# kartikmadhira1/YA_VO

Hardware: AMD Instinct MI355X
Metric: frames/sec (detect+describe+match+PnP) on 1241×376 KITTI stereo; RMSE vs CPU ref (higher is better)
Workload: dtype u8

## Files before the change

ya_vo_amd/csrc/yavo_kernels.hip:

```cpp
#include <hip/hip_runtime.h>
#include <stdint.h>
#include <stdlib.h>
#include <string.h>

#include <algorithm>

#include "yavo_xlane.h"
#include "yavo_internal.h"


namespace yavo {

__device__ __forceinline__ int lane_id() { return (int)(threadIdx.x & 63); }

__device__ __forceinline__ int wave_incl_scan(int v) {
    v += __builtin_amdgcn_update_dpp(0, v, 0x111, 0xf, 0xf, false);
    v += __builtin_amdgcn_update_dpp(0, v, 0x112, 0xf, 0xf, false);
    v += __builtin_amdgcn_update_dpp(0, v, 0x114, 0xf, 0xf, false);
    v += __builtin_amdgcn_update_dpp(0, v, 0x118, 0xf, 0xf, false);
    v += __builtin_amdgcn_update_dpp(0, v, 0x142, 0xa, 0xf, false);
    v += __builtin_amdgcn_update_dpp(0, v, 0x143, 0xc, 0xf, false);
    return v;
}

// ... 162 lines not shown
    return kw;
}

__device__ __forceinline__ int reflect101(int p, int len) {
    if (p < 0) p = -p;
    if (p >= len) p = 2 * len - p - 2;
    return p;
}

#ifdef YAVO_LM_PROFILE
constexpr int kDetProfSlots = 131072;
__device__ unsigned long long g_det_prof[kDetProfSlots][6];
#define DP_DECL unsigned long long dp_acc[6] = {0, 0, 0, 0, 0, 0}; unsigned long long dp_t = __builtin_readcyclecounter();
#define DP_MARK(k) do { const unsigned long long t_ = __builtin_readcyclecounter(); dp_acc[k] += t_ - dp_t; dp_t = t_; } while (0)
#define DP_STORE() do { \
        const unsigned slot_ = blockIdx.x; \
        if (threadIdx.x == 0 && slot_ < kDetProfSlots) for (int q_ = 0; q_ < 6; ++q_) g_det_prof[slot_][q_] = dp_acc[q_]; \
    } while (0)
constexpr int kBriefProfSlots = 16384;
__device__ unsigned long long g_brief_prof[kBriefProfSlots][6];
#define BP_DECL unsigned long long bp_acc[3] = {0, 0, 0}; unsigned long long bp_t = __builtin_readcyclecounter(); \
    unsigned long long bp_bands = 0; const unsigned long long bp_rt0 = __builtin_amdgcn_s_memrealtime();
#define BP_MARK(k) do { const unsigned long long t_ = __builtin_readcyclecounter(); bp_acc[k] += t_ - bp_t; bp_t = t_; } while (0)
#define BP_BAND() do { ++bp_bands; } while (0)
#define BP_STORE() do { \
        if (threadIdx.x == 0 && blockIdx.x < kBriefProfSlots) { \
            g_brief_prof[blockIdx.x][0] = bp_acc[0]; g_brief_prof[blockIdx.x][1] = bp_acc[1]; \
            g_brief_prof[blockIdx.x][2] = bp_rt0; \
            g_brief_prof[blockIdx.x][3] = __builtin_amdgcn_s_memrealtime(); \
            g_brief_prof[blockIdx.x][4] = (unsigned long long)__builtin_amdgcn_s_getreg(0xF804) | (bp_bands << 32); \
            g_brief_prof[blockIdx.x][5] = (unsigned long long)__builtin_amdgcn_s_getreg(0xF814) | (bp_acc[2] << 32); \
        } \
    } while (0)
#else
#define DP_DECL
#define DP_MARK(k) do {} while (0)
#define DP_STORE() do {} while (0)
#define BP_DECL
#define BP_MARK(k) do {} while (0)
#define BP_BAND() do {} while (0)
#define BP_STORE() do {} while (0)
#endif
constexpr int FT_W = kFastTileW;
constexpr int FT_H = kFastTileH;
constexpr int FT_R = 4;
constexpr int FT_LW = FT_W + 2 * FT_R;
constexpr int FT_LH = FT_H + 2 * FT_R;
constexpr int kBandM = 19;
constexpr int kBlurStageDw = FT_LH * (FT_W / 4);

__device__ __forceinline__ void blur_tile_mfma(const uint8_t* tile, const uint32_t* s_band, uint32_t* stage, int hbias,
                                               int lane, int cb) {
    typedef int dt_v4i __attribute__((ext_vector_type(4)));
    const int nn = lane & 15, g = lane >> 4;
    const uint32_t* band = &s_band[(nn & 3) * kBandM + 3 - (nn >> 2)];
    const dt_v4i B = {(int)band[4 * g], (int)band[4 * g + 1], (int)band[4 * g + 2], (int)band[4 * g + 3]};
    const dt_v4i Z = {0, 0, 0, 0};
    const uint8_t* arow = &tile[nn * FT_LW + 16 * cb + 16 * g];
    dt_v4i Hlo, Hhi;
#pragma unroll
    for (int rb = 0; rb < 4; ++rb) {
        const uint2 lo = *reinterpret_cast<const uint2*>(arow + 16 * rb * FT_LW);
        const uint2 hi = *reinterpret_cast<const uint2*>(arow + 16 * rb * FT_LW + 8);
        const dt_v4i A = {(int)(lo.x ^ 0x80808080u), (int)(lo.y ^ 0x80808080u), (int)(hi.x ^ 0x80808080u),
                          (int)(hi.y ^ 0x80808080u)};
        const dt_v4i acc = __builtin_amdgcn_mfma_i32_16x16x64_i8(A, B, Z, 0, 0, 0);
        const uint32_t p01 = __builtin_amdgcn_perm((uint32_t)acc[1], (uint32_t)acc[0], 0x05010400u);
        const uint32_t p23 = __builtin_amdgcn_perm((uint32_t)acc[3], (uint32_t)acc[2], 0x05010400u);
        Hlo[rb] = (int)(__builtin_amdgcn_perm(p23, p01, 0x05040100u) ^ 0x80808080u);
        Hhi[rb] = (int)__builtin_amdgcn_perm(p23, p01, 0x07060302u);
// ... 280 lines not shown
    for (int rr = ty; rr < BL_H; rr += 4) {
        const int r = r0 + rr;
        uint32_t acc = 0;
#pragma unroll
        for (int i = 0; i < 9; ++i) acc += kw.k[i] * th[(rr + i) * BL_W + tx];
        uint32_t v = (acc + (1u << 15)) >> 16;
        if (r < H && c < W) blur[(int64_t)img * blur_image_bytes(H, W) + (int64_t)r * blur_pitch(W) + c] = (uint8_t)(v > 255u ? 255u : v);
    }
}

void launch_blur9(const uint8_t* imgs, int n_images, int H, int W, int stride, int64_t pitch,
                  const uint16_t* k9_host, uint8_t* blur, hipStream_t s) {
    const K9 kw = make_k9(k9_host);
    constexpr int kMaxGridZ = 65535;
    for (int i0 = 0; i0 < n_images; i0 += kMaxGridZ) {
        const int n = n_images - i0 < kMaxGridZ ? n_images - i0 : kMaxGridZ;
        dim3 grid((W + BL_W - 1) / BL_W, (H + BL_H - 1) / BL_H, n);
        hipLaunchKernelGGL(blur9_kernel, grid, dim3(256), 0, s, imgs + (int64_t)i0 * pitch, H, W, stride, pitch, kw,
                           blur + (int64_t)i0 * blur_image_bytes(H, W));
    }
}

constexpr int TK_NT = 1024;

__device__ __forceinline__ bool brief_boundary(int row, int col, int H, int W) {
    return !(col - 8 < 0 || col + 8 > W) && !(row - 8 < 0 || row + 8 > H);
}

__host__ __device__ constexpr int bank_classes(int nb) { return nb <= kBandCounters / 32 ? 32 : 1; }

template <int NT, class RcAt>
__device__ void boundary_compact(RcAt rc_at, int K, int H, int W, int32_t* kp_src, int32_t* kp_count,
                                 int32_t* kp_band, int32_t* band_off, int* s_tmp, int* s_band) {
    const int tid = threadIdx.x;
    const int nb = (H + kBandRows - 1) / kBandRows;
    const int C = bank_classes(nb), nbc = nb * C;
    const int LS = brief_lds_stride(W);
    auto bucket = [&](int row, int col) -> int {
        const int band = row / kBandRows;
        const int cls = C == 1 ? 0 : ((((row - band * kBandRows + 8) * LS + col) >> 2) & 31);
        return band * C + cls;
    };
    for (int b = tid; b < nbc; b += NT) s_band[b] = 0;
    __syncthreads();
    int base = 0;
    for (int pass = 0; pass < 2; ++pass) {
        base = 0;
        for (int c0 = 0; c0 < K; c0 += 4 * NT) {
            int flags[4];
            int2 rcs[4];
            int cnt = 0;
#pragma unroll
            for (int u = 0; u < 4; ++u) {
                const int i = c0 + tid * 4 + u;
                flags[u] = 0;
                rcs[u] = make_int2(0, 0);
                if (i < K) {
                    rcs[u] = rc_at(i);
                    flags[u] = brief_boundary(rcs[u].x, rcs[u].y, H, W) ? 1 : 0;
                }
                cnt += flags[u];
            }
            int total = 0;
            int off = base + block_excl_scan<NT>(cnt, s_tmp, &total);
#pragma unroll
            for (int u = 0; u < 4; ++u) {
                const int i = c0 + tid * 4 + u;
                if (flags[u]) {
                    const int bk = bucket(rcs[u].x, rcs[u].y);
                    if (pass == 0) {
                        reinterpret_cast<int4*>(kp_src)[off] = make_int4(rcs[u].x, rcs[u].y, i, 0);
                        atomicAdd(&s_band[bk], 1);
                    } else {
                        const int pos = atomicAdd(&s_band[bk], 1);
                        reinterpret_cast<int4*>(kp_band)[pos] = make_int4(rcs[u].x, rcs[u].y, i, off);
                    }
                    off++;
                }
            }
            base += total;
        }
        __syncthreads();
        if (pass == 0) {
            int acc = 0;
            for (int b0 = 0; b0 < nbc; b0 += NT) {
                const int j = b0 + tid;
                const int c = j < nbc ? s_band[j] : 0;
                int tot = 0;
                const int first = acc + block_excl_scan<NT>(c, s_tmp, &tot);
                if (j < nbc) {
                    s_band[j] = first;
                    if (j % C == 0) band_off[j / C] = first;
                }
                acc += tot;
            }
            if (tid == 0) band_off[nb] = acc;
        }
        __syncthreads();
    }
    if (tid == 0) *kp_count = base;
}

constexpr int TK_SEL_NT = 512;
static_assert(TK_SEL_NT >= 256 && TK_SEL_NT % 64 == 0, "the radix-select histogram scan uses the first 256 threads");
template <int NT>
__global__ __launch_bounds__(NT) void topk_kernel(const uint64_t* __restrict__ cand_keys, int64_t cap,
                                                     uint32_t* __restrict__ cand_count, uint32_t* __restrict__ cand_seen,
                                                     int H, int W, int max_kp, int keep, int32_t* __restrict__ det_rc,
                                                     float* __restrict__ det_resp, int32_t* __restrict__ det_count,
                                                     int32_t* __restrict__ kp_src, int32_t* __restrict__ kp_count,
                                                     int32_t* __restrict__ kp_band, int32_t* __restrict__ band_off,
                                                     int32_t* __restrict__ brief_heads) {
    __shared__ uint64_t s_keys[kMaxKp];
    __shared__ uint32_t s_hist[256];
    __shared__ int s_tmp[40];
    __shared__ int s_band[kBandCounters];
    __shared__ uint64_t s_prefix, s_mask;
    __shared__ int s_krem, s_done, s_n;

    const int img = blockIdx.x;
    const int tid = threadIdx.x;
    if (img == 0 && tid < kBriefHeads) brief_heads[tid] = 0;
    const uint64_t* keys = cand_keys + (int64_t)img * cap;
    int64_t C64 = (int64_t)cand_count[img];
    if (C64 > cap) C64 = cap;
    const int C = (int)C64;
    const int K = C < keep ? C : keep;
    __syncthreads();
    if (tid == 0) {
        cand_seen[img] = (uint32_t)C;
        cand_count[img] = 0;
    }
    int32_t* rc_out = det_rc + (int64_t)img * max_kp * 2;
    float* resp_out = det_resp + (int64_t)img * max_kp;

    if (K == 0) {
        const int nb = (H + kBandRows - 1) / kBandRows;
        for (int b = tid; b <= nb; b += NT) band_off[(int64_t)img * (kMaxBands + 1) + b] = 0;
        if (tid == 0) { det_count[img] = 0; kp_count[img] = 0; }
        return;
    }
    uint64_t sel_mask = 0, sel_prefix = ~0ull;
    if (C > K) {
        if (tid == 0) { s_prefix = 0; s_mask = 0; s_krem = K; s_done = 0; }
        __syncthreads();
        for (int shift = 56; shift >= 0; shift -= 8) {
            const uint64_t pm = s_mask, pp = s_prefix;
            const int krem = s_krem;
            if (tid < 256) s_hist[tid] = 0;
            __syncthreads();
            for (int i = tid; i < C; i += NT) {
                const uint64_t k = keys[i];
                if ((k & pm) == pp) atomicAdd(&s_hist[(k >> shift) & 255u], 1u);
            }
            __syncthreads();
            int h = 0, incl = 0;
            if (tid < 256) {
                h = (int)s_hist[tid];
                incl = wave_incl_scan(h);
                if ((tid & 63) == 63) s_tmp[tid >> 6] = incl;
            }
            __syncthreads();
            if (tid < 256) {
                int base = 0;
                for (int w = 0; w < (tid >> 6); ++w) base += s_tmp[w];
                incl += base;
                if (incl >= krem && incl - h < krem) {
                    const int nk = krem - (incl - h);
                    s_prefix = pp | ((uint64_t)tid << shift);
                    s_mask = pm | (0xFFull << shift);
                    s_krem = nk;
                    s_done = (h == nk);
                }
            }
            __syncthreads();
            if (s_done) break;
        }
        sel_mask = s_mask;
        sel_prefix = s_prefix;
    }
    if (tid == 0) s_n = 0;
    __syncthreads();
    for (int i = tid; i < C; i += NT) {
        const uint64_t k = keys[i];
        if ((k & sel_mask) <= sel_prefix) {
            const int p = atomicAdd(&s_n, 1);
            if (p < kMaxKp) s_keys[p] = k;
        }
    }
    __syncthreads();
    int P2 = 1;
    while (P2 < K) P2 <<= 1;
    for (int i = K + tid; i < P2; i += NT) s_keys[i] = ~0ull;
    __syncthreads();
    for (int size = 2; size <= P2; size <<= 1) {
        for (int stride = size >> 1; stride > 0; stride >>= 1) {
            for (int t = tid; t < (P2 >> 1); t += NT) {
                const int i = 2 * t - (t & (stride - 1));
                const int j = i + stride;
                const bool up = ((i & size) == 0);
                const uint64_t a = s_keys[i], b = s_keys[j];
                if ((a > b) == up) { s_keys[i] = b; s_keys[j] = a; }
            }
            __syncthreads();
        }
    }
    for (int i = tid; i < K; i += NT) {
        const uint64_t k = s_keys[i];
        const uint32_t idx = (uint32_t)k;
        const int row = (int)(idx / (uint32_t)W), col = (int)(idx - (uint32_t)row * (uint32_t)W);
        rc_out[2 * i] = row;
        rc_out[2 * i + 1] = col;
        resp_out[i] = key_resp(k);
    }
    if (tid == 0) det_count[img] = K;
    const uint32_t Wu = (uint32_t)W;
    auto rc_from_lds = [&](int i) -> int2 {
        const uint32_t idx = (uint32_t)s_keys[i];
        const uint32_t row = idx / Wu;
        return make_int2((int)row, (int)(idx - row * Wu));
    };
    boundary_compact<NT>(rc_from_lds, K, H, W, kp_src + (int64_t)img * max_kp * 4, kp_count + img,
                         kp_band + (int64_t)img * max_kp * 4, band_off + (int64_t)img * (kMaxBands + 1), s_tmp, s_band);
}

__global__ __launch_bounds__(TK_NT) void kp_boundary_kernel(const int32_t* __restrict__ det_rc,
                                                            const int32_t* __restrict__ det_count, int H, int W,
                                                            int max_kp, int32_t* __restrict__ kp_src,
                                                            int32_t* __restrict__ kp_count, int32_t* __restrict__ kp_band,
                                                            int32_t* __restrict__ band_off,
                                                            int32_t* __restrict__ brief_heads) {
    __shared__ int s_tmp[40];
    __shared__ int s_band[kBandCounters];
    const int img = blockIdx.x;
    if (img == 0 && threadIdx.x < kBriefHeads) brief_heads[threadIdx.x] = 0;
    int K = det_count[img];
    if (K > max_kp) K = max_kp;
    const int32_t* rc = det_rc + (int64_t)img * max_kp * 2;
    auto rc_from_global = [&](int i) -> int2 { return make_int2(rc[2 * i], rc[2 * i + 1]); };
    boundary_compact<TK_NT>(rc_from_global, K, H, W, kp_src + (int64_t)img * max_kp * 4, kp_count + img,
                            kp_band + (int64_t)img * max_kp * 4, band_off + (int64_t)img * (kMaxBands + 1), s_tmp,
                            s_band);
}

void launch_topk(const uint64_t* cand_keys, int64_t cap, uint32_t* cand_count, uint32_t* cand_seen, int n_images,
                 int H, int W, int max_kp, int keep, int32_t* det_rc, float* det_resp, int32_t* det_count, int32_t* kp_src,
                 int32_t* kp_count, int32_t* kp_band, int32_t* band_off, int32_t* brief_heads, hipStream_t s) {
    hipLaunchKernelGGL(topk_kernel<TK_SEL_NT>, dim3(n_images), dim3(TK_SEL_NT), 0, s, cand_keys, cap, cand_count,
                       cand_seen, H, W, max_kp, keep, det_rc, det_resp, det_count, kp_src, kp_count, kp_band, band_off,
                       brief_heads);
}

void launch_kp_boundary(const int32_t* det_rc, const int32_t* det_count, int n_images, int H, int W, int max_kp,
                        int32_t* kp_src, int32_t* kp_count, int32_t* kp_band, int32_t* band_off, int32_t* brief_heads,
                        hipStream_t s) {
    hipLaunchKernelGGL(kp_boundary_kernel, dim3(n_images), dim3(TK_NT), 0, s, det_rc, det_count, H, W, max_kp,
                       kp_src, kp_count, kp_band, band_off, brief_heads);
}


constexpr int BR_BAND = kBandRows;
constexpr int BR_ROWS = BR_BAND + 17;
constexpr int BR_NT = 1024;
constexpr int BR_NW = BR_NT / 64;
static_assert(4 * BR_NT >= kMaxKp, "brief_kernel loads at most 4 * BR_NT band records");

__device__ __forceinline__ int brief_take(int32_t* heads, int label, int total, int& at) {
    const int q = total >> 3, r = total & 7;
    while (at < kBriefHeads) {
        const int x = (label + at) & 7;
        const int len = q + (x < r ? 1 : 0);
        if (len > 0) {
            const int v = atomicAdd(&heads[x], 1);
            if (v < len) return (x < r ? x * (q + 1) : r * (q + 1) + (x - r) * q) + v;
        }
        ++at;
    }
    return -1;
}

// ... 861 lines not shown
        const int i = tid * 4 + u;
        flags[u] = (i < n && (int)src[(int64_t)i * REC_DW + 24] < lim) ? 1 : 0;
        cnt += flags[u];
    }
    int total = 0;
    int off = block_excl_scan<FZ_NT>(cnt, s_tmp, &total);
#pragma unroll
    for (int u = 0; u < 4; ++u) {
        const int i = tid * 4 + u;
        if (i < n) s_pos[i] = flags[u] ? off : -1;
        off += flags[u];
    }
    __syncthreads();
    uint32_t* dst = reinterpret_cast<uint32_t*>(out);
    for (int dw = tid; dw < n * REC_DW; dw += FZ_NT) {
        const int i = dw / REC_DW;
        const int f = dw - i * REC_DW;
        const int p = s_pos[i];
        if (p < 0) continue;
        uint32_t v = src[dw];
        if (f == 3 || f == 15) v = (v & ~0xFFu) | 1u;
        dst[(int64_t)p * REC_DW + f] = v;
    }
    if (tid == 0) *out_count = total;
}

void launch_filter_records(const yv_match* in, int n, int thr, yv_match* out, int32_t* out_count, hipStream_t s) {
    hipLaunchKernelGGL(filter_records_kernel, dim3(1), dim3(FZ_NT), 0, s, in, n, thr, out, out_count);
}

}

#ifdef YAVO_LM_PROFILE
extern "C" int yv_debug_brief_prof(unsigned long long* out ) {
    return hipMemcpyFromSymbol(out, HIP_SYMBOL(yavo::g_brief_prof), sizeof(unsigned long long) * 16384 * 6) ==
                   hipSuccess ? 0 : -2;
}
extern "C" int yv_debug_det_prof(unsigned long long* out ) {
    return hipMemcpyFromSymbol(out, HIP_SYMBOL(yavo::g_det_prof), sizeof(unsigned long long) * 131072 * 6) ==
                   hipSuccess ? 0 : -2;
}
#endif

namespace yavo {
__global__ void xlane_check_kernel(int32_t* out) {
    const int l = threadIdx.x;
    out[0 * 64 + l] = xl::xor_row_i32<1>(l);
    out[1 * 64 + l] = xl::xor_row_i32<2>(l);
    out[2 * 64 + l] = xl::xor_row_i32<4>(l);
    out[3 * 64 + l] = xl::xor_row_i32<8>(l);
    uint32_t a = (uint32_t)l, b = 100u + (uint32_t)l;
    xl::swap_halves<16>(a, b);
    out[4 * 64 + l] = (int32_t)a;
    out[5 * 64 + l] = (int32_t)b;
    a = (uint32_t)l;
    b = 100u + (uint32_t)l;
    xl::swap_halves<32>(a, b);
    out[6 * 64 + l] = (int32_t)a;
    out[7 * 64 + l] = (int32_t)b;
}
}

extern "C" int yv_debug_xlane(int32_t* d_out , void* stream) {
    if (!d_out) return -1;
    hipLaunchKernelGGL(yavo::xlane_check_kernel, dim3(1), dim3(64), 0, reinterpret_cast<hipStream_t>(stream), d_out);
    return hipGetLastError() == hipSuccess ? 0 : -2;
}
```

Baseline: 255,700.

## Add register-resident fast top-k kernel with wave-level radix select and bitonic sort

Adds a topk_fast_kernel that holds up to 16 candidate keys per thread in registers. It narrows the radix select with wave OR/AND reductions over the high key bits, builds per-wave ballot-peeled histograms, sorts four keys per thread with in-register cross-lane bitonic stages that go through LDS only for large strides, and fuses the boundary compaction and band scan. Its goal is to cut the many LDS passes and syncthreads of the generic shared-memory bitonic sort and select. Images with too many candidates fall back to the refactored general path. This adds a large amount of code and register pressure, with an occupancy attribute pinned to 8 waves per EU.

```diff
diff --git a/ya_vo_amd/csrc/yavo_kernels.hip b/ya_vo_amd/csrc/yavo_kernels.hip
--- a/ya_vo_amd/csrc/yavo_kernels.hip
+++ b/ya_vo_amd/csrc/yavo_kernels.hip
@@ -218,7 +218,22 @@
             g_brief_prof[blockIdx.x][5] = (unsigned long long)__builtin_amdgcn_s_getreg(0xF814) | (bp_acc[2] << 32); \
         } \
     } while (0)
+constexpr int kTopkProfSlots = 8192;
+__device__ unsigned long long g_topk_prof[kTopkProfSlots][8];
+#define TP_DECL unsigned long long tp_acc[6] = {0, 0, 0, 0, 0, 0}; unsigned long long tp_t = __builtin_readcyclecounter(); \
+    const unsigned long long tp_rt0 = __builtin_amdgcn_s_memrealtime();
+#define TP_MARK(k) do { const unsigned long long t_ = __builtin_readcyclecounter(); tp_acc[k] += t_ - tp_t; tp_t = t_; } while (0)
+#define TP_STORE() do { \
+        if (threadIdx.x == 0 && blockIdx.x < kTopkProfSlots) { \
+            for (int q_ = 0; q_ < 6; ++q_) g_topk_prof[blockIdx.x][q_] = tp_acc[q_]; \
+            g_topk_prof[blockIdx.x][6] = tp_rt0; \
+            g_topk_prof[blockIdx.x][7] = __builtin_amdgcn_s_memrealtime(); \
+        } \
+    } while (0)
 #else
+#define TP_DECL
+#define TP_MARK(k) do {} while (0)
+#define TP_STORE() do {} while (0)
 #define DP_DECL
 #define DP_MARK(k) do {} while (0)
 #define DP_STORE() do {} while (0)
@@ -640,19 +655,15 @@
 constexpr int TK_SEL_NT = 512;
 static_assert(TK_SEL_NT >= 256 && TK_SEL_NT % 64 == 0, "the radix-select histogram scan uses the first 256 threads");
 template <int NT>
-__global__ __launch_bounds__(NT) void topk_kernel(const uint64_t* __restrict__ cand_keys, int64_t cap,
-                                                     uint32_t* __restrict__ cand_count, uint32_t* __restrict__ cand_seen,
-                                                     int H, int W, int max_kp, int keep, int32_t* __restrict__ det_rc,
-                                                     float* __restrict__ det_resp, int32_t* __restrict__ det_count,
-                                                     int32_t* __restrict__ kp_src, int32_t* __restrict__ kp_count,
-                                                     int32_t* __restrict__ kp_band, int32_t* __restrict__ band_off,
-                                                     int32_t* __restrict__ brief_heads) {
-    __shared__ uint64_t s_keys[kMaxKp];
-    __shared__ uint32_t s_hist[256];
-    __shared__ int s_tmp[40];
-    __shared__ int s_band[kBandCounters];
-    __shared__ uint64_t s_prefix, s_mask;
-    __shared__ int s_krem, s_done, s_n;
+__device__ void topk_general(const uint64_t* __restrict__ cand_keys, int64_t cap, uint32_t* __restrict__ cand_count,
+                             uint32_t* __restrict__ cand_seen, int H, int W, int max_kp, int keep,
+                             int32_t* __restrict__ det_rc, float* __restrict__ det_resp,
+                             int32_t* __restrict__ det_count, int32_t* __restrict__ kp_src,
+                             int32_t* __restrict__ kp_count, int32_t* __restrict__ kp_band,
+                             int32_t* __restrict__ band_off, int32_t* __restrict__ brief_heads, uint64_t* s_keys,
+                             int key_cap, uint32_t* s_hist, int* s_tmp, int* s_band, uint64_t* s_state, int* s_ctl) {
+    uint64_t &s_prefix = s_state[0], &s_mask = s_state[1];
+    int &s_krem = s_ctl[0], &s_done = s_ctl[1], &s_n = s_ctl[2];
 
     const int img = blockIdx.x;
     const int tid = threadIdx.x;
@@ -721,7 +732,7 @@
         const uint64_t k = keys[i];
         if ((k & sel_mask) <= sel_prefix) {
             const int p = atomicAdd(&s_n, 1);
-            if (p < kMaxKp) s_keys[p] = k;
+            if (p < key_cap) s_keys[p] = k;
         }
     }
     __syncthreads();
@@ -758,6 +769,434 @@
     };
     boundary_compact<NT>(rc_from_lds, K, H, W, kp_src + (int64_t)img * max_kp * 4, kp_count + img,
                          kp_band + (int64_t)img * max_kp * 4, band_off + (int64_t)img * (kMaxBands + 1), s_tmp, s_band);
+}
+
+template <int NT>
+__global__ __launch_bounds__(NT) void topk_kernel(const uint64_t* __restrict__ cand_keys, int64_t cap,
+                                                     uint32_t* __restrict__ cand_count, uint32_t* __restrict__ cand_seen,
+                                                     int H, int W, int max_kp, int keep, int32_t* __restrict__ det_rc,
+                                                     float* __restrict__ det_resp, int32_t* __restrict__ det_count,
+                                                     int32_t* __restrict__ kp_src, int32_t* __restrict__ kp_count,
+                                                     int32_t* __restrict__ kp_band, int32_t* __restrict__ band_off,
+                                                     int32_t* __restrict__ brief_heads) {
+    __shared__ uint64_t s_keys[kMaxKp];
+    __shared__ uint32_t s_hist[256];
+    __shared__ int s_tmp[40];
+    __shared__ int s_band[kBandCounters];
+    __shared__ uint64_t s_state[2];
+    __shared__ int s_ctl[3];
+    topk_general<NT>(cand_keys, cap, cand_count, cand_seen, H, W, max_kp, keep, det_rc, det_resp, det_count, kp_src,
+                     kp_count, kp_band, band_off, brief_heads, s_keys, kMaxKp, s_hist, s_tmp, s_band, s_state, s_ctl);
+}
+
+constexpr int TKF_NT = 512;
+constexpr int TKF_R = 16;
+constexpr int TKF_CAP = TKF_NT * TKF_R;
+constexpr int TKF_MAXK = 4 * TKF_NT;
+constexpr int TKF_PEEL = 1;
+static_assert(TKF_NT * 16 == 8 * 256 * 4, "one 16-byte store per thread zeroes the eight histograms");
+static_assert(kBandCounters <= 2 * TKF_NT, "two (band, class) counters per thread");
+static_assert(kBriefHeads <= TKF_NT, "the band queue's heads are zeroed by one thread each");
+
+__device__ __forceinline__ uint64_t tk_u64(uint32_t lo, uint32_t hi) { return ((uint64_t)hi << 32) | lo; }
+
+__device__ __forceinline__ void tk_cx(uint64_t& a, uint64_t& b, bool up) {
+    const bool sw = (a > b) == up;
+    const uint64_t t = sw ? b : a;
+    b = sw ? a : b;
+    a = t;
+}
+
+template <int M>
+__device__ __forceinline__ void tk_lane_cx(uint64_t& k, bool keep_min) {
+    const uint32_t lo = (uint32_t)k, hi = (uint32_t)(k >> 32);
+    uint64_t a, b;
+    if constexpr (M < 16) {
+        a = k;
+        b = tk_u64(xl::xor_row<M>(lo), xl::xor_row<M>(hi));
+    } else {
+        uint32_t alo = lo, blo = lo, ahi = hi, bhi = hi;
+        xl::swap_halves<M>(alo, blo);
+        xl::swap_halves<M>(ahi, bhi);
+        a = tk_u64(alo, ahi);
+        b = tk_u64(blo, bhi);
+    }
+    k = ((a < b) == keep_min) ? a : b;
+}
+
+template <int STRIDE>
+__device__ __forceinline__ void tk_stage(uint64_t (&k)[4], bool up, int tid) {
+    if constexpr (STRIDE == 1) {
+        tk_cx(k[0], k[1], up);
+        tk_cx(k[2], k[3], up);
+    } else if constexpr (STRIDE == 2) {
+        tk_cx(k[0], k[2], up);
+        tk_cx(k[1], k[3], up);
+    } else {
+        constexpr int M = STRIDE / 4;
+        const bool keep_min = ((tid & M) == 0) == up;
+#pragma unroll
+        for (int j = 0; j < 4; ++j) tk_lane_cx<M>(k[j], keep_min);
+    }
+}
+template <int STRIDE>
+__device__ __forceinline__ void tk_merge(uint64_t (&k)[4], bool up, int tid) {
+    tk_stage<STRIDE>(k, up, tid);
+    if constexpr (STRIDE > 1) tk_merge<STRIDE / 2>(k, up, tid);
+}
+template <int SIZE>
+__device__ __forceinline__ void tk_sort_levels(uint64_t (&k)[4], int tid) {
+    if constexpr (SIZE == 2) {
+        tk_cx(k[0], k[1], true);
+        tk_cx(k[2], k[3], false);
+    } else {
+        tk_sort_levels<SIZE / 2>(k, tid);
+        tk_merge<SIZE / 2>(k, ((4 * tid) & SIZE) == 0, tid);
+    }
+}
+
+__device__ __forceinline__ uint32_t tk_wave_or(uint32_t v) {
+    v |= xl::xor_row<1>(v);
+    v |= xl::xor_row<2>(v);
+    v |= xl::xor_row<4>(v);
+    v |= xl::xor_row<8>(v);
+    uint32_t x = v, y = v;
+    xl::swap_halves<16>(x, y);
+    v = x | y;
+    x = y = v;
+    xl::swap_halves<32>(x, y);
+    return x | y;
+}
+
+__device__ __forceinline__ int tk_prefix_popc(uint64_t m) {
+    return (int)__builtin_amdgcn_mbcnt_hi((uint32_t)(m >> 32), __builtin_amdgcn_mbcnt_lo((uint32_t)m, 0u));
+}
+
+__device__ __forceinline__ void tk_hist_add(uint32_t* hist, uint32_t dg, bool act, int lane) {
+    bool pend = act;
+    if constexpr (TKF_PEEL > 0) {
+        uint64_t rem = __ballot(pend);
+#pragma unroll
+        for (int it = 0; it < TKF_PEEL; ++it) {
+            if (!rem) break;
+            const int src = __builtin_ctzll(rem);
+            const uint32_t d0 = (uint32_t)__builtin_amdgcn_readlane((int)dg, src);
+            const uint64_t same = __ballot(pend && dg == d0);
+            if (lane == src) atomicAdd(&hist[d0], (uint32_t)__builtin_popcountll(same));
+            pend = pend && dg != d0;
+            rem &= ~same;
+        }
+    }
+    if (pend) atomicAdd(&hist[dg], 1u);
+}
+template <bool LOW>
+__device__ __forceinline__ void tk_hist_pass(const uint64_t (&k)[TKF_R], uint32_t phi, uint32_t m, uint32_t p, int sh,
+                                             uint32_t* hist, int lane) {
+#pragma unroll
+    for (int r = 0; r < TKF_R; ++r) {
+        const uint32_t hi = (uint32_t)(k[r] >> 32), lo = (uint32_t)k[r];
+        const uint32_t w = LOW ? lo : hi;
+        const bool act = (w & m) == p && (!LOW || hi == phi);
+        tk_hist_add(hist, (w >> sh) & 255u, act, lane);
+    }
+}
+__device__ __forceinline__ void tk_find_bucket(const uint32_t* hist, int lane, int krem, int& bin, int& hh,
+                                               int& before) {
+    const uint4 h4 = reinterpret_cast<const uint4*>(hist)[lane];
+    const int h[4] = {(int)h4.x, (int)h4.y, (int)h4.z, (int)h4.w};
+    const int sum = h[0] + h[1] + h[2] + h[3];
+    const int incl = wave_incl_scan(sum);
+    int run = incl - sum, b = 0, c = 0, bf = 0;
+    const bool mine = run < krem && krem <= incl;
+#pragma unroll
+    for (int q = 0; q < 4; ++q) {
+        if (run < krem && krem <= run + h[q]) { b = 4 * lane + q; c = h[q]; bf = run; }
+        run += h[q];
+    }
+    const int src = __builtin_ctzll(__ballot(mine));
+    bin = __builtin_amdgcn_readlane(b, src);
+    hh = __builtin_amdgcn_readlane(c, src);
+    before = __builtin_amdgcn_readlane(bf, src);
+}
+
+#define TKF_OCCUPANCY __attribute__((amdgpu_waves_per_eu(8, 8)))
+template <int NT>
+__global__ __launch_bounds__(NT) TKF_OCCUPANCY void topk_fast_kernel(
+    const uint64_t* __restrict__ cand_keys, int64_t cap, uint32_t* __restrict__ cand_count,
+    uint32_t* __restrict__ cand_seen, int H, int W, int max_kp, int keep, int32_t* __restrict__ det_rc,
+    float* __restrict__ det_resp, int32_t* __restrict__ det_count, int32_t* __restrict__ kp_src,
+    int32_t* __restrict__ kp_count, int32_t* __restrict__ kp_band, int32_t* __restrict__ band_off,
+    int32_t* __restrict__ brief_heads, int force_general) {
+    static_assert(NT == TKF_NT, "the register layouts are written for 512 threads");
+    constexpr int NW = NT / 64;
+    __shared__ __attribute__((aligned(16))) uint64_t s_buf[2][TKF_MAXK];
+    __shared__ __attribute__((aligned(16))) int s_band[kBandCounters];
+    __shared__ __attribute__((aligned(16))) int s_tmp[40];
+    __shared__ uint64_t s_state[2];
+    __shared__ int s_ctl[3];
+    uint32_t* const s_hist = reinterpret_cast<uint32_t*>(s_buf[1]);
+
+    const int img = blockIdx.x;
+    const int tid = threadIdx.x, lane = tid & 63, wave = tid >> 6;
+    int64_t C64 = (int64_t)cand_count[img];
+    if (C64 > cap) C64 = cap;
+    const int C = (int)C64;
+    if (force_general || C > TKF_CAP) {
+        topk_general<NT>(cand_keys, cap, cand_count, cand_seen, H, W, max_kp, keep, det_rc, det_resp, det_count, kp_src,
+                         kp_count, kp_band, band_off, brief_heads, s_buf[0], TKF_MAXK, s_hist, s_tmp, s_band, s_state,
+                         s_ctl);
+        return;
+    }
+    const int K = C < keep ? C : keep;
+    if (img == 0 && tid < kBriefHeads) brief_heads[tid] = 0;
+    const int nb = (H + kBandRows - 1) / kBandRows;
+    int32_t* const boff = band_off + (int64_t)img * (kMaxBands + 1);
+    if (K == 0) {
+        __syncthreads();
+        for (int b = tid; b <= nb; b += NT) boff[b] = 0;
+        if (tid == 0) { cand_seen[img] = (uint32_t)C; cand_count[img] = 0; det_count[img] = 0; kp_count[img] = 0; }
+        return;
+    }
+
+    TP_DECL
+    const uint64_t* keys = cand_keys + (int64_t)img * cap;
+    uint64_t k[TKF_R];
+#pragma unroll
+    for (int r = 0; r < TKF_R; ++r) {
+        const int i = r * NT + tid;
+        k[r] = i < C ? keys[i] : ~0ull;
+    }
+    const int NC = bank_classes(nb), nbc = nb * NC;
+    reinterpret_cast<uint4*>(s_hist)[tid] = make_uint4(0u, 0u, 0u, 0u);
+    reinterpret_cast<uint4*>(s_buf[0])[2 * tid] = make_uint4(~0u, ~0u, ~0u, ~0u);
+    reinterpret_cast<uint4*>(s_buf[0])[2 * tid + 1] = make_uint4(~0u, ~0u, ~0u, ~0u);
+    for (int b = tid; b < nbc; b += NT) s_band[b] = 0;
+    if (tid == 0) s_ctl[2] = 0;
+    int P2 = 256;
+    while (P2 < K) P2 <<= 1;
+    const bool cut = C > P2;
+    if (cut) {
+        uint32_t o0 = 0u, a0 = ~0u, o1 = 0u, a1 = ~0u;
+        int n0 = 0;
+#pragma unroll
+        for (int r = 0; r < TKF_R; ++r) {
+            const uint32_t hi = (uint32_t)(k[r] >> 32);
+            const bool v = r * NT + tid < C, neg = (hi >> 31) != 0u;
+            n0 += __builtin_popcountll(__ballot(v && !neg));
+            o0 |= v && !neg ? hi : 0u;
+            a0 &= v && !neg ? hi : ~0u;
+            o1 |= v && neg ? hi : 0u;
+            a1 &= v && neg ? hi : ~0u;
+        }
+        o0 = tk_wave_or(o0);
+        a0 = ~tk_wave_or(~a0);
+        o1 = tk_wave_or(o1);
+        a1 = ~tk_wave_or(~a1);
+        if (lane == 0) {
+            int* t = s_tmp + 5 * wave;
+            t[0] = n0; t[1] = (int)o0; t[2] = (int)a0; t[3] = (int)o1; t[4] = (int)a1;
+        }
+    }
+    __syncthreads();
+    if (tid == 0) {
+        cand_seen[img] = (uint32_t)C;
+        cand_count[img] = 0;
+    }
+
+    TP_MARK(0);
+    uint64_t sel_mask = 0, sel_prefix = ~0ull;
+    if (cut) {
+        int n0 = 0;
+        uint32_t o0 = 0u, a0 = ~0u, o1 = 0u, a1 = ~0u;
+#pragma unroll
+        for (int w = 0; w < NW; ++w) {
+            const int* t = s_tmp + 5 * w;
+            n0 += t[0]; o0 |= (uint32_t)t[1]; a0 &= (uint32_t)t[2]; o1 |= (uint32_t)t[3]; a1 &= (uint32_t)t[4];
+        }
+        const bool c1 = K > n0;
+        int krem = __builtin_amdgcn_readfirstlane(c1 ? K - n0 : K);
+        const uint32_t orc = __builtin_amdgcn_readfirstlane(c1 ? o1 : o0);
+        const uint32_t andc = __builtin_amdgcn_readfirstlane(c1 ? a1 : a0);
+        const uint32_t diff = orc & ~andc;
+        const int hbh = diff ? 31 - __builtin_clz(diff) : -1;
+        uint32_t mhi = diff ? ~0u << (hbh + 1) : ~0u;
+        uint32_t phi = andc & mhi;
+        uint32_t mlo = 0u, plo = 0u;
+        int pass = 0, bin, hh, before, M;
+        bool done = false;
+        if (diff) {
+            for (int sh = hbh > 7 ? hbh - 7 : 0;; sh = sh > 8 ? sh - 8 : 0) {
+                uint32_t* hist = s_hist + 256 * pass++;
+                tk_hist_pass<false>(k, 0u, mhi, phi, sh, hist, lane);
+                __syncthreads();
+                tk_find_bucket(hist, lane, krem, bin, hh, before);
+                krem -= before;
+                phi |= (uint32_t)bin << sh;
+                mhi |= 0xFFu << sh;
+                M = K - krem + hh;
+                done = M <= P2;
+                if (done || sh == 0) break;
+            }
+        }
+        if (!done) {
+            for (int sh = 24;; sh = sh > 8 ? sh - 8 : 0) {
+                uint32_t* hist = s_hist + 256 * pass++;
+                tk_hist_pass<true>(k, phi, mlo, plo, sh, hist, lane);
+                __syncthreads();
+                tk_find_bucket(hist, lane, krem, bin, hh, before);
+                krem -= before;
+                plo |= (uint32_t)bin << sh;
+                mlo |= 0xFFu << sh;
+                M = K - krem + hh;
+                if (M <= P2 || sh == 0) break;
+            }
+        }
+        sel_mask = tk_u64(mlo, mhi);
+        sel_prefix = tk_u64(plo, phi);
+    }
+
+    TP_MARK(1);
+    {
+        uint32_t selbits = 0;
+        int wtot = 0;
+#pragma unroll
+        for (int r = 0; r < TKF_R; ++r) {
+            const bool s = (r * NT + tid < C) && (k[r] & sel_mask) <= sel_prefix;
+            selbits |= (s ? 1u : 0u) << r;
+            wtot += __builtin_popcountll(__ballot(s));
+        }
+        int base = 0;
+        if (lane == 0) base = atomicAdd(&s_ctl[2], wtot);
+        base = __builtin_amdgcn_readfirstlane(base);
+#pragma unroll
+        for (int r = 0; r < TKF_R; ++r) {
+            const bool s = (selbits >> r) & 1u;
+            const uint64_t bal = __ballot(s);
+            const int pos = base + tk_prefix_popc(bal);
+            if (s && pos < TKF_MAXK) s_buf[0][pos] = k[r];
+            base += __builtin_popcountll(bal);
+        }
+    }
+    __syncthreads();
+
+    TP_MARK(2);
+    uint64_t q[4] = {~0ull, ~0ull, ~0ull, ~0ull};
+    const bool live = 4 * tid < P2;
+    if (live) {
+        const uint4 a = reinterpret_cast<const uint4*>(s_buf[0])[2 * tid];
+        const uint4 b = reinterpret_cast<const uint4*>(s_buf[0])[2 * tid + 1];
+        q[0] = tk_u64(a.x, a.y); q[1] = tk_u64(a.z, a.w); q[2] = tk_u64(b.x, b.y); q[3] = tk_u64(b.z, b.w);
+        tk_sort_levels<256>(q, tid);
+    }
+    TP_MARK(3);
+    int cur = 1;
+    for (int size = 512; size <= P2; size <<= 1) {
+        const bool up = ((4 * tid) & size) == 0;
+        for (int stride = size >> 1; stride >= 256; stride >>= 1) {
+            if (live) {
+                uint4* dst = reinterpret_cast<uint4*>(s_buf[cur]) + 2 * tid;
+                dst[0] = make_uint4((uint32_t)q[0], (uint32_t)(q[0] >> 32), (uint32_t)q[1], (uint32_t)(q[1] >> 32));
+                dst[1] = make_uint4((uint32_t)q[2], (uint32_t)(q[2] >> 32), (uint32_t)q[3], (uint32_t)(q[3] >> 32));
+            }
+            __syncthreads();
+            if (live) {
+                const uint4* src = reinterpret_cast<const uint4*>(s_buf[cur]) + (((4 * tid) ^ stride) >> 1);
+                const uint4 a = src[0], b = src[1];
+                const uint64_t p[4] = {tk_u64(a.x, a.y), tk_u64(a.z, a.w), tk_u64(b.x, b.y), tk_u64(b.z, b.w)};
+                const bool keep_min = (((4 * tid) & stride) == 0) == up;
+#pragma unroll
+                for (int j = 0; j < 4; ++j) {
+                    q[j] = ((q[j] < p[j]) == keep_min) ? q[j] : p[j];
+                }
+            }
+            cur ^= 1;
+        }
+        if (live) tk_merge<128>(q, up, tid);
+    }
+
+    TP_MARK(4);
+    int32_t* rc_out = det_rc + (int64_t)img * max_kp * 2;
+    float* resp_out = det_resp + (int64_t)img * max_kp;
+    const uint32_t Wu = (uint32_t)W;
+    const int LS = brief_lds_stride(W);
+    int2 rcs[4];
+    int flags[4];
+    int cnt = 0;
+#pragma unroll
+    for (int j = 0; j < 4; ++j) {
+        const int i = 4 * tid + j;
+        flags[j] = 0;
+        rcs[j] = make_int2(0, 0);
+        if (i < K) {
+            const uint32_t idx = (uint32_t)q[j];
+            const uint32_t row = idx / Wu;
+            rcs[j] = make_int2((int)row, (int)(idx - row * Wu));
+            reinterpret_cast<int2*>(rc_out)[i] = rcs[j];
+            resp_out[i] = key_resp(q[j]);
+            flags[j] = brief_boundary(rcs[j].x, rcs[j].y, H, W) ? 1 : 0;
+        }
+        cnt += flags[j];
+    }
+    if (tid == 0) det_count[img] = K;
+    const int incl = wave_incl_scan(cnt);
+    if (lane == 63) s_tmp[8 + wave] = incl;
+    __syncthreads();
+    int off = incl - cnt, total = 0;
+#pragma unroll
+    for (int w = 0; w < NW; ++w) {
+        const int t = s_tmp[8 + w];
+        off += w < wave ? t : 0;
+        total += t;
+    }
+    int32_t* src_out = kp_src + (int64_t)img * max_kp * 4;
+    int32_t* band_out = kp_band + (int64_t)img * max_kp * 4;
+    int bks[4];
+#pragma unroll
+    for (int j = 0, o = off; j < 4; ++j) {
+        bks[j] = 0;
+        if (flags[j]) {
+            const int row = rcs[j].x, col = rcs[j].y;
+            const int band = row / kBandRows;
+            const int cls = NC == 1 ? 0 : ((((row - band * kBandRows + 8) * LS + col) >> 2) & 31);
+            bks[j] = band * NC + cls;
+            reinterpret_cast<int4*>(src_out)[o] = make_int4(row, col, 4 * tid + j, 0);
+            atomicAdd(&s_band[bks[j]], 1);
+            ++o;
+        }
+    }
+    __syncthreads();
+    {
+        const int j0 = 2 * tid;
+        const int c0 = j0 < nbc ? s_band[j0] : 0, c1 = j0 + 1 < nbc ? s_band[j0 + 1] : 0;
+        const int s = c0 + c1;
+        const int inc2 = wave_incl_scan(s);
+        if (lane == 63) s_tmp[16 + wave] = inc2;
+        __syncthreads();
+        int first = inc2 - s;
+#pragma unroll
+        for (int w = 0; w < NW; ++w) first += w < wave ? s_tmp[16 + w] : 0;
+        if (j0 < nbc) {
+            s_band[j0] = first;
+            if (j0 % NC == 0) boff[j0 / NC] = first;
+        }
+        if (j0 + 1 < nbc) {
+            s_band[j0 + 1] = first + c0;
+            if ((j0 + 1) % NC == 0) boff[(j0 + 1) / NC] = first + c0;
+        }
+        if (tid == 0) boff[nb] = total;
+    }
+    __syncthreads();
+#pragma unroll
+    for (int j = 0, o = off; j < 4; ++j) {
+        if (flags[j]) {
+            const int pos = atomicAdd(&s_band[bks[j]], 1);
+            reinterpret_cast<int4*>(band_out)[pos] = make_int4(rcs[j].x, rcs[j].y, 4 * tid + j, o);
+            ++o;
+        }
+    }
+    if (tid == 0) kp_count[img] = total;
+    TP_MARK(5);
+    TP_STORE();
 }
 
 __global__ __launch_bounds__(TK_NT) void kp_boundary_kernel(const int32_t* __restrict__ det_rc,
@@ -779,9 +1218,17 @@
                             s_band);
 }
 
+static int g_topk_path = 0;
+
 void launch_topk(const uint64_t* cand_keys, int64_t cap, uint32_t* cand_count, uint32_t* cand_seen, int n_images,
                  int H, int W, int max_kp, int keep, int32_t* det_rc, float* det_resp, int32_t* det_count, int32_t* kp_src,
                  int32_t* kp_count, int32_t* kp_band, int32_t* band_off, int32_t* brief_heads, hipStream_t s) {
+    if (max_kp <= TKF_MAXK && g_topk_path != 1) {
+        hipLaunchKernelGGL(topk_fast_kernel<TKF_NT>, dim3(n_images), dim3(TKF_NT), 0, s, cand_keys, cap, cand_count,
+                           cand_seen, H, W, max_kp, keep, det_rc, det_resp, det_count, kp_src, kp_count, kp_band,
+                           band_off, brief_heads, g_topk_path == 2 ? 1 : 0);
+        return;
+    }
     hipLaunchKernelGGL(topk_kernel<TK_SEL_NT>, dim3(n_images), dim3(TK_SEL_NT), 0, s, cand_keys, cap, cand_count,
                        cand_seen, H, W, max_kp, keep, det_rc, det_resp, det_count, kp_src, kp_count, kp_band, band_off,
                        brief_heads);
@@ -1709,6 +2156,10 @@
 }
 
 #ifdef YAVO_LM_PROFILE
+extern "C" int yv_debug_topk_prof(unsigned long long* out ) {
+    return hipMemcpyFromSymbol(out, HIP_SYMBOL(yavo::g_topk_prof), sizeof(unsigned long long) * 8192 * 8) ==
+                   hipSuccess ? 0 : -2;
+}
 extern "C" int yv_debug_brief_prof(unsigned long long* out ) {
     return hipMemcpyFromSymbol(out, HIP_SYMBOL(yavo::g_brief_prof), sizeof(unsigned long long) * 16384 * 6) ==
                    hipSuccess ? 0 : -2;
@@ -1718,6 +2169,13 @@
                    hipSuccess ? 0 : -2;
 }
 #endif
+
+extern "C" int yv_debug_set_topk_path(void* ctx, int mode) {
+    if (!ctx || mode < 0 || mode > 2) return -1;
+    yavo::g_topk_path = mode;
+    return 0;
+}
+extern "C" int yv_debug_topk_capacity(void) { return yavo::TKF_CAP; }
 
 namespace yavo {
 __global__ void xlane_check_kernel(int32_t* out) {
```

Result: no change. 257,400 (median of 3 runs) (+0.7%).

## Stage top-k radix select in LDS with adaptive bit passes and wave-aggregated compaction

Applied to the files above, without the earlier changes.

When the candidate count fits, the top-k select copies the 32-bit response keys into LDS once. It then runs the radix histogram passes from LDS, using AND/OR reductions to skip constant bits, rather than rereading global keys for every byte. Candidate gathering now uses one ballot-based atomic per wave instead of one atomic per thread. boundary_compact keeps its points in registers so it does not rerun the first pass, and sorted keys are repacked as row<<16|col to avoid integer division. The costs are more register and LDS pressure, extra profiling macros, and a fallback path for inputs too large to stage.

```diff
diff --git a/ya_vo_amd/csrc/yavo_kernels.hip b/ya_vo_amd/csrc/yavo_kernels.hip
--- a/ya_vo_amd/csrc/yavo_kernels.hip
+++ b/ya_vo_amd/csrc/yavo_kernels.hip
@@ -218,10 +218,20 @@
             g_brief_prof[blockIdx.x][5] = (unsigned long long)__builtin_amdgcn_s_getreg(0xF814) | (bp_acc[2] << 32); \
         } \
     } while (0)
+constexpr int kTopkProfSlots = 16384;
+__device__ unsigned long long g_topk_prof[kTopkProfSlots][5];
+#define TP_DECL unsigned long long tp_acc[5] = {0, 0, 0, 0, 0}; unsigned long long tp_t = __builtin_readcyclecounter();
+#define TP_MARK(k) do { const unsigned long long t_ = __builtin_readcyclecounter(); tp_acc[k] += t_ - tp_t; tp_t = t_; } while (0)
+#define TP_STORE() do { \
+        if (threadIdx.x == 0 && blockIdx.x < kTopkProfSlots) for (int q_ = 0; q_ < 5; ++q_) g_topk_prof[blockIdx.x][q_] = tp_acc[q_]; \
+    } while (0)
 #else
 #define DP_DECL
 #define DP_MARK(k) do {} while (0)
 #define DP_STORE() do {} while (0)
+#define TP_DECL
+#define TP_MARK(k) do {} while (0)
+#define TP_STORE() do {} while (0)
 #define BP_DECL
 #define BP_MARK(k) do {} while (0)
 #define BP_BAND() do {} while (0)
@@ -568,6 +578,8 @@
 template <int NT, class RcAt>
 __device__ void boundary_compact(RcAt rc_at, int K, int H, int W, int32_t* kp_src, int32_t* kp_count,
                                  int32_t* kp_band, int32_t* band_off, int* s_tmp, int* s_band) {
+    constexpr int NCH = (kMaxKp + 4 * NT - 1) / (4 * NT);
+    static_assert(NCH <= 2, "a thread keeps the points of all its chunks in registers");
     const int tid = threadIdx.x;
     const int nb = (H + kBandRows - 1) / kBandRows;
     const int C = bank_classes(nb), nbc = nb * C;
@@ -579,62 +591,73 @@
     };
     for (int b = tid; b < nbc; b += NT) s_band[b] = 0;
     __syncthreads();
+    int2 rcs[NCH][4];
+    int offs[NCH];
+    uint32_t flags = 0;
     int base = 0;
-    for (int pass = 0; pass < 2; ++pass) {
-        base = 0;
-        for (int c0 = 0; c0 < K; c0 += 4 * NT) {
-            int flags[4];
-            int2 rcs[4];
-            int cnt = 0;
-#pragma unroll
-            for (int u = 0; u < 4; ++u) {
-                const int i = c0 + tid * 4 + u;
-                flags[u] = 0;
-                rcs[u] = make_int2(0, 0);
-                if (i < K) {
-                    rcs[u] = rc_at(i);
-                    flags[u] = brief_boundary(rcs[u].x, rcs[u].y, H, W) ? 1 : 0;
+#pragma unroll
+    for (int ch = 0; ch < NCH; ++ch) {
+        const int c0 = ch * 4 * NT;
+        offs[ch] = 0;
+#pragma unroll
+        for (int u = 0; u < 4; ++u) rcs[ch][u] = make_int2(0, 0);
+        if (c0 >= K) continue;
+        int cnt = 0;
+#pragma unroll
+        for (int u = 0; u < 4; ++u) {
+            const int i = c0 + tid * 4 + u;
+            if (i < K) {
+                rcs[ch][u] = rc_at(i);
+                if (brief_boundary(rcs[ch][u].x, rcs[ch][u].y, H, W)) {
+                    flags |= 1u << (4 * ch + u);
+                    ++cnt;
                 }
-                cnt += flags[u];
-            }
-            int total = 0;
-            int off = base + block_excl_scan<NT>(cnt, s_tmp, &total);
-#pragma unroll
-            for (int u = 0; u < 4; ++u) {
-                const int i = c0 + tid * 4 + u;
-                if (flags[u]) {
-                    const int bk = bucket(rcs[u].x, rcs[u].y);
-                    if (pass == 0) {
-                        reinterpret_cast<int4*>(kp_src)[off] = make_int4(rcs[u].x, rcs[u].y, i, 0);
-                        atomicAdd(&s_band[bk], 1);
-                    } else {
-                        const int pos = atomicAdd(&s_band[bk], 1);
-                        reinterpret_cast<int4*>(kp_band)[pos] = make_int4(rcs[u].x, rcs[u].y, i, off);
-                    }
-                    off++;
-                }
-            }
-            base += total;
-        }
-        __syncthreads();
-        if (pass == 0) {
-            int acc = 0;
-            for (int b0 = 0; b0 < nbc; b0 += NT) {
-                const int j = b0 + tid;
-                const int c = j < nbc ? s_band[j] : 0;
-                int tot = 0;
-                const int first = acc + block_excl_scan<NT>(c, s_tmp, &tot);
-                if (j < nbc) {
-                    s_band[j] = first;
-                    if (j % C == 0) band_off[j / C] = first;
-                }
-                acc += tot;
-            }
-            if (tid == 0) band_off[nb] = acc;
-        }
-        __syncthreads();
-    }
-    if (tid == 0) *kp_count = base;
+            }
+        }
+        int total = 0;
+        int off = base + block_excl_scan<NT>(cnt, s_tmp, &total);
+        offs[ch] = off;
+#pragma unroll
+        for (int u = 0; u < 4; ++u) {
+            if (flags & (1u << (4 * ch + u))) {
+                reinterpret_cast<int4*>(kp_src)[off] = make_int4(rcs[ch][u].x, rcs[ch][u].y, c0 + tid * 4 + u, 0);
+                atomicAdd(&s_band[bucket(rcs[ch][u].x, rcs[ch][u].y)], 1);
+                off++;
+            }
+        }
+        base += total;
+    }
+    __syncthreads();
+    int acc = 0;
+    for (int b0 = 0; b0 < nbc; b0 += NT) {
+        const int j = b0 + tid;
+        const int c = j < nbc ? s_band[j] : 0;
+        int tot = 0;
+        const int first = acc + block_excl_scan<NT>(c, s_tmp, &tot);
+        if (j < nbc) {
+            s_band[j] = first;
+            if (j % C == 0) band_off[j / C] = first;
+        }
+        acc += tot;
+    }
+    if (tid == 0) {
+        band_off[nb] = acc;
+        *kp_count = base;
+    }
+    __syncthreads();
+#pragma unroll
+    for (int ch = 0; ch < NCH; ++ch) {
+        int off = offs[ch];
+#pragma unroll
+        for (int u = 0; u < 4; ++u) {
+            if (flags & (1u << (4 * ch + u))) {
+                const int pos = atomicAdd(&s_band[bucket(rcs[ch][u].x, rcs[ch][u].y)], 1);
+                reinterpret_cast<int4*>(kp_band)[pos] =
+                    make_int4(rcs[ch][u].x, rcs[ch][u].y, ch * 4 * NT + tid * 4 + u, off);
+                off++;
+            }
+        }
+    }
 }
 
 constexpr int TK_SEL_NT = 512;
@@ -650,12 +673,18 @@
     __shared__ uint64_t s_keys[kMaxKp];
     __shared__ uint32_t s_hist[256];
     __shared__ int s_tmp[40];
-    __shared__ int s_band[kBandCounters];
+    __shared__ __align__(16) int s_band[kBandCounters];
     __shared__ uint64_t s_prefix, s_mask;
     __shared__ int s_krem, s_done, s_n;
+    __shared__ uint32_t s_and, s_or;
+    constexpr int kStaged = 2 * kMaxKp;
+    static_assert(kBandCounters == 4 * 256, "s_band holds the staged select's four histograms");
 
     const int img = blockIdx.x;
     const int tid = threadIdx.x;
+    TP_DECL
+    if (tid == 0) { s_n = 0; s_and = ~0u; s_or = 0u; }
+    for (int j = tid; j < kBandCounters; j += NT) s_band[j] = 0;
     if (img == 0 && tid < kBriefHeads) brief_heads[tid] = 0;
     const uint64_t* keys = cand_keys + (int64_t)img * cap;
     int64_t C64 = (int64_t)cand_count[img];
@@ -674,54 +703,150 @@
         const int nb = (H + kBandRows - 1) / kBandRows;
         for (int b = tid; b <= nb; b += NT) band_off[(int64_t)img * (kMaxBands + 1) + b] = 0;
         if (tid == 0) { det_count[img] = 0; kp_count[img] = 0; }
+        TP_STORE();
         return;
     }
     uint64_t sel_mask = 0, sel_prefix = ~0ull;
     if (C > K) {
-        if (tid == 0) { s_prefix = 0; s_mask = 0; s_krem = K; s_done = 0; }
-        __syncthreads();
-        for (int shift = 56; shift >= 0; shift -= 8) {
-            const uint64_t pm = s_mask, pp = s_prefix;
-            const int krem = s_krem;
-            if (tid < 256) s_hist[tid] = 0;
+        uint64_t pm0 = 0, pp0 = 0;
+        int krem0 = K, shift0 = 56;
+        bool done = false;
+        if (C <= kStaged) {
+            uint32_t* s_resp = reinterpret_cast<uint32_t*>(s_keys);
+            uint32_t* s_h4 = reinterpret_cast<uint32_t*>(s_band);
+            const int lane = lane_id();
+            uint32_t pm = 0, pp = 0, rem = 0;
+            int krem = K;
+            auto pick = [&](const uint32_t* hist, int sh) {
+                const uint4 h4 = reinterpret_cast<const uint4*>(hist)[lane];
+                const int sum = (int)(h4.x + h4.y + h4.z + h4.w);
+                const int incl = wave_incl_scan(sum);
+                int below = incl - sum;
+                const bool hit = below < krem && krem <= incl;
+                int bin = 4 * lane, h = (int)h4.x;
+                if (below + h < krem) { below += h; ++bin; h = (int)h4.y; }
+                if (below + h < krem) { below += h; ++bin; h = (int)h4.z; }
+                if (below + h < krem) { below += h; ++bin; h = (int)h4.w; }
+                const int src = __ffsll((unsigned long long)__ballot(hit)) - 1;
+                bin = __shfl(bin, src);
+                h = __shfl(h, src);
+                below = __shfl(below, src);
+                pp |= (uint32_t)bin << sh;
+                pm |= 255u << sh;
+                krem -= below;
+                done = (h == krem);
+            };
+            uint32_t all_and = ~0u, all_or = 0u;
+            for (int i0 = 0; i0 < C; i0 += 8 * NT) {
+                uint64_t k[8];
+#pragma unroll
+                for (int u = 0; u < 8; ++u) {
+                    const int i = i0 + u * NT + tid;
+                    k[u] = i < C ? keys[i] : 0ull;
+                }
+#pragma unroll
+                for (int u = 0; u < 8; ++u) {
+                    const int i = i0 + u * NT + tid;
+                    const uint32_t r = (uint32_t)(k[u] >> 32);
+                    if (i < C) {
+                        s_resp[i] = r;
+                        all_and &= r;
+                        all_or |= r;
+                        atomicAdd(&s_h4[r >> 24], 1u);
+                    }
+                }
+            }
+            all_and &= xl::xor_row<1>(all_and); all_or |= xl::xor_row<1>(all_or);
+            all_and &= xl::xor_row<2>(all_and); all_or |= xl::xor_row<2>(all_or);
+            all_and &= xl::xor_row<4>(all_and); all_or |= xl::xor_row<4>(all_or);
+            all_and &= xl::xor_row<8>(all_and); all_or |= xl::xor_row<8>(all_or);
+            if ((tid & 15) == 0) {
+                atomicAnd(&s_and, all_and);
+                atomicOr(&s_or, all_or);
+            }
             __syncthreads();
-            for (int i = tid; i < C; i += NT) {
-                const uint64_t k = keys[i];
-                if ((k & pm) == pp) atomicAdd(&s_hist[(k >> shift) & 255u], 1u);
-            }
+            pick(s_h4, 24);
+            rem = (s_and ^ s_or) & 0x00FFFFFFu;
+            for (int pass = 1; rem != 0 && !done; ++pass) {
+                const int hib = 31 - __clz((int)rem);
+                const int sh = hib >= 7 ? hib - 7 : 0;
+                uint32_t* hist = s_h4 + 256 * pass;
+                for (int i = tid; i < C; i += NT) {
+                    const uint32_t r = s_resp[i];
+                    if ((r & pm) == pp) atomicAdd(&hist[(r >> sh) & 255u], 1u);
+                }
+                __syncthreads();
+                pick(hist, sh);
+                rem &= (1u << sh) - 1u;
+            }
+            pm0 = (uint64_t)pm << 32;
+            pp0 = (uint64_t)pp << 32;
+            krem0 = krem;
+            shift0 = 24;
+        }
+        sel_mask = pm0;
+        sel_prefix = pp0;
+        if (!done) {
+            if (tid == 0) { s_prefix = pp0; s_mask = pm0; s_krem = krem0; s_done = 0; }
             __syncthreads();
-            int h = 0, incl = 0;
-            if (tid < 256) {
-                h = (int)s_hist[tid];
-                incl = wave_incl_scan(h);
-                if ((tid & 63) == 63) s_tmp[tid >> 6] = incl;
-            }
-            __syncthreads();
-            if (tid < 256) {
+            for (int shift = shift0; shift >= 0; shift -= 8) {
+                const uint64_t pm = s_mask, pp = s_prefix;
+                const int krem = s_krem;
+                if (tid < 256) s_hist[tid] = 0;
+                __syncthreads();
+                for (int i = tid; i < C; i += NT) {
+                    const uint64_t k = keys[i];
+                    if ((k & pm) == pp) atomicAdd(&s_hist[(k >> shift) & 255u], 1u);
+                }
+                __syncthreads();
+                int h = 0, incl = 0;
+                if (tid < 256) {
+                    h = (int)s_hist[tid];
+                    incl = wave_incl_scan(h);
+                    if ((tid & 63) == 63) s_tmp[tid >> 6] = incl;
+                }
+                __syncthreads();
+                if (tid < 256) {
+                    int base = 0;
+                    for (int w = 0; w < (tid >> 6); ++w) base += s_tmp[w];
+                    incl += base;
+                    if (incl >= krem && incl - h < krem) {
+                        const int nk = krem - (incl - h);
+                        s_prefix = pp | ((uint64_t)tid << shift);
+                        s_mask = pm | (0xFFull << shift);
+                        s_krem = nk;
+                        s_done = (h == nk);
+                    }
+                }
+                __syncthreads();
+                if (s_done) break;
+            }
+            sel_mask = s_mask;
+            sel_prefix = s_prefix;
+        }
+    }
+    TP_MARK(0);
+    {
+        const int lane = lane_id();
+        for (int i0 = 0; i0 < C; i0 += 4 * NT) {
+            uint64_t k[4];
+#pragma unroll
+            for (int u = 0; u < 4; ++u) {
+                const int i = i0 + u * NT + tid;
+                k[u] = i < C ? keys[i] : ~0ull;
+            }
+#pragma unroll
+            for (int u = 0; u < 4; ++u) {
+                const bool sel = i0 + u * NT + tid < C && (k[u] & sel_mask) <= sel_prefix;
+                const unsigned long long bal = __ballot(sel);
+                if (bal == 0) continue;
+                const int leader = __ffsll(bal) - 1;
                 int base = 0;
-                for (int w = 0; w < (tid >> 6); ++w) base += s_tmp[w];
-                incl += base;
-                if (incl >= krem && incl - h < krem) {
-                    const int nk = krem - (incl - h);
-                    s_prefix = pp | ((uint64_t)tid << shift);
-                    s_mask = pm | (0xFFull << shift);
-                    s_krem = nk;
-                    s_done = (h == nk);
-                }
-            }
-            __syncthreads();
-            if (s_done) break;
-        }
-        sel_mask = s_mask;
-        sel_prefix = s_prefix;
-    }
-    if (tid == 0) s_n = 0;
-    __syncthreads();
-    for (int i = tid; i < C; i += NT) {
-        const uint64_t k = keys[i];
-        if ((k & sel_mask) <= sel_prefix) {
-            const int p = atomicAdd(&s_n, 1);
-            if (p < kMaxKp) s_keys[p] = k;
+                if (lane == leader) base = atomicAdd(&s_n, __popcll(bal));
+                base = __shfl(base, leader);
+                const int p = base + __popcll(bal & ((1ull << lane) - 1ull));
+                if (sel && p < kMaxKp) s_keys[p] = k[u];
+            }
         }
     }
     __syncthreads();
@@ -729,6 +854,7 @@
     while (P2 < K) P2 <<= 1;
     for (int i = K + tid; i < P2; i += NT) s_keys[i] = ~0ull;
     __syncthreads();
+    TP_MARK(1);
     for (int size = 2; size <= P2; size <<= 1) {
         for (int stride = size >> 1; stride > 0; stride >>= 1) {
             for (int t = tid; t < (P2 >> 1); t += NT) {
@@ -741,6 +867,7 @@
             __syncthreads();
         }
     }
+    TP_MARK(2);
     for (int i = tid; i < K; i += NT) {
         const uint64_t k = s_keys[i];
         const uint32_t idx = (uint32_t)k;
@@ -748,16 +875,19 @@
         rc_out[2 * i] = row;
         rc_out[2 * i + 1] = col;
         resp_out[i] = key_resp(k);
+        s_keys[i] = (k & 0xFFFFFFFF00000000ull) | (uint32_t)(row << 16 | col);
     }
     if (tid == 0) det_count[img] = K;
-    const uint32_t Wu = (uint32_t)W;
+    TP_MARK(3);
+    static_assert(kBandRows * kMaxBands <= 65536 && kMaxWidth <= 65536, "row << 16 | col");
     auto rc_from_lds = [&](int i) -> int2 {
-        const uint32_t idx = (uint32_t)s_keys[i];
-        const uint32_t row = idx / Wu;
-        return make_int2((int)row, (int)(idx - row * Wu));
+        const uint32_t v = (uint32_t)s_keys[i];
+        return make_int2((int)(v >> 16), (int)(v & 0xFFFFu));
     };
     boundary_compact<NT>(rc_from_lds, K, H, W, kp_src + (int64_t)img * max_kp * 4, kp_count + img,
                          kp_band + (int64_t)img * max_kp * 4, band_off + (int64_t)img * (kMaxBands + 1), s_tmp, s_band);
+    TP_MARK(4);
+    TP_STORE();
 }
 
 __global__ __launch_bounds__(TK_NT) void kp_boundary_kernel(const int32_t* __restrict__ det_rc,
@@ -1713,6 +1843,10 @@
     return hipMemcpyFromSymbol(out, HIP_SYMBOL(yavo::g_brief_prof), sizeof(unsigned long long) * 16384 * 6) ==
                    hipSuccess ? 0 : -2;
 }
+extern "C" int yv_debug_topk_prof(unsigned long long* out ) {
+    return hipMemcpyFromSymbol(out, HIP_SYMBOL(yavo::g_topk_prof), sizeof(unsigned long long) * 16384 * 5) ==
+                   hipSuccess ? 0 : -2;
+}
 extern "C" int yv_debug_det_prof(unsigned long long* out ) {
     return hipMemcpyFromSymbol(out, HIP_SYMBOL(yavo::g_det_prof), sizeof(unsigned long long) * 131072 * 6) ==
                    hipSuccess ? 0 : -2;
```

Result: no change. 255,800 before, 256,700 after, median of 6 (+0.4%).
